# paulvantieghem/curla

Measured on AMD Instinct MI355X. Metric: SAC+CURL gradient updates/sec, batch=512 84x84x9, higher is better.
Workload: dtype f32

## Files before the change

curla_amd/_lib.py:

```python
import ctypes
import os

_HERE = os.path.dirname(os.path.abspath(__file__))
LIB_PATH = os.environ.get("CURLA_LIB_PATH") or os.path.join(_HERE, "libcurla_hip.so")

c_int, c_ll, c_float, c_size_t, vp = ctypes.c_int, ctypes.c_longlong, ctypes.c_float, ctypes.c_size_t, ctypes.c_void_p
c_u64 = ctypes.c_ulonglong
c_double = ctypes.c_double

ABI_VERSION = 8

SIGNATURES = {
    "curla_conv1_fwd": [vp, c_int, vp, vp, vp, vp, vp, vp, c_int, c_int, c_int, c_int, c_int, c_int, c_int, c_float, vp],
    "curla_conv3x3_s1_fwd": [vp, vp, vp, vp, c_int, c_int, c_int, c_int, vp],
    "curla_conv3x3_s1_fwd2": [vp, vp, vp, vp, c_int, vp, vp, vp, vp, c_int, c_int, c_int, c_int, vp],
    "curla_conv3x3_s1_fwd_stack": [c_int, vp, vp, vp, vp, c_int, vp, vp, vp, vp, c_int, c_int, c_int, c_int, vp],
    "curla_conv3x3_s1_stack_granule": [],
    "curla_conv1_fwd2": [vp, vp, vp, vp, vp, vp, vp, c_int, vp, vp, vp, vp, vp, vp, c_int, c_int, c_int, c_int, c_int, c_int,
                         c_int, c_float, vp],
    "curla_conv3x3_s1_dgrad": [vp, vp, vp, vp, c_int, c_int, c_int, c_int, vp],
    "curla_conv3x3_s1_wgrad": [vp, vp, vp, vp, vp, c_int, c_int, c_int, c_int, vp],
    "curla_conv1_wgrad": [vp, c_int, vp, vp, vp, vp, vp, vp, vp, c_int, c_int, c_int, c_int, c_int, c_int, c_int,
                          c_float, vp],
    "curla_conv3x3_s1_wgrad_slabs": [vp, vp, vp, c_int, c_int, c_int, c_int, vp, vp],
# ... 13 lines not shown
    "curla_fc_bwd_ln2": [vp, vp, vp, vp, vp, c_int, c_int, c_int, vp, c_int, vp, vp, vp, vp, c_int, c_int, vp, vp],
    "curla_curl_head": [vp, vp, vp, vp, vp, vp, c_int, c_int, vp, vp, vp, vp, vp, vp, vp, vp, vp, vp],
    "curla_gemm_nested": [vp, c_int, c_int, c_ll, c_ll, vp, c_int, c_int, c_ll, c_ll, vp, c_int, c_ll, c_ll, c_int, c_int, c_int,
                          c_int, c_int, c_float, vp, c_ll, c_ll, c_int, vp, c_int, c_ll, c_ll, vp],
    "curla_mlp_out_fwd_nested": [vp, c_ll, c_ll, vp, c_ll, c_ll, vp, c_ll, c_ll, vp, c_ll, c_ll, c_int, c_int, c_int, c_int, c_int,
                                 vp],
    "curla_gemm_multi": [c_int, vp, vp, vp, c_int, c_int, c_int, c_int, c_int, c_int, c_int, c_ll, vp],
    "curla_fc_fwd_multi": [c_int, vp, vp, vp, c_int, c_int, c_int, c_int, c_ll, c_int, vp],
    "curla_splitk_reduce": [vp, c_int, c_ll, c_int, c_int, c_int, vp, c_int, vp, c_int, vp],
    "curla_mlp_out_fwd": [vp, c_ll, vp, c_ll, vp, c_ll, vp, c_ll, c_int, c_int, c_int, c_int, vp],
    "curla_mlp_out_bwd": [vp, c_ll, vp, c_ll, vp, c_ll, vp, c_ll, vp, c_ll, c_int, c_int, c_int, c_int, vp],
    "curla_mlp_out_bwd_loss": [vp, vp, c_ll, vp, c_ll, vp, c_ll, vp, c_ll, c_int, c_int, vp, vp, c_ll, vp],
    "curla_mlp_out_bwd_bias": [vp, c_ll, vp, c_ll, vp, c_ll, vp, c_ll, vp, c_ll, c_int, c_int, c_int, c_int, vp, vp, c_ll,
                               vp],
    "curla_gemm_small_shape": [c_int, c_int, c_int, c_int],
    "curla_gemm_colsum": [vp, c_int, c_int, c_ll, vp, c_int, c_int, c_ll, vp, c_int, c_ll, c_int, c_int, c_int, c_int, vp,
                          c_ll, vp],
    "curla_linear_bwd": [vp, c_ll, vp, c_ll, vp, c_ll, vp, c_ll, vp, c_ll, vp, c_ll, vp, c_ll, c_int, c_int, c_int, c_int, vp],
    "curla_fc_ln_fwd": [vp, c_int, c_ll, c_int, vp, vp, vp, c_int, c_int, c_float, vp, vp, vp, vp, c_int, vp, vp, c_int,
                        vp],
    "curla_critic_td_loss": [vp, vp, c_ll, vp, vp, vp, vp, c_float, c_int, vp, vp, vp, vp],
    "curla_soft_update2": [vp, vp, c_size_t, c_size_t, c_float, c_float, c_float, c_float, vp],
    "curla_adam_step": [vp, vp, vp, vp, c_size_t, c_double, c_double, c_double, c_double, c_ll, vp, vp],
    "curla_adam_step_lerp": [vp, vp, vp, vp, c_size_t, c_double, c_double, c_double, c_double, c_ll, vp, vp, c_size_t,
                             c_float, c_float, c_float, c_float, vp],
    "curla_adam_step_scalar64": [vp, vp, vp, vp, c_size_t, c_double, c_double, c_double, c_double, c_ll, vp, vp, vp, vp, vp,
                                 c_double, c_double, c_double, c_double, c_ll, vp, vp],
    "curla_adam_step2": [vp, vp, vp, vp, vp, vp, c_size_t, c_size_t, c_double, c_double, c_double, c_double, c_ll, c_double,
                         c_double, c_double, c_double, c_ll, vp, vp],
    "curla_f64_pack": [vp, vp, vp],
# ... 27 lines not shown
    "curla_stage_frames_u8": [vp, vp, c_ll, c_int, c_int, c_int, c_int, c_int, c_int, c_int, c_int, vp],
    "curla_gather_stacks": [vp, vp, c_int, vp, c_int, c_int, c_int, c_int, vp, vp],
    "curla_nhwc_to_nchw": [vp, vp, c_int, c_int, c_int, c_int, vp],
    "curla_color_jiggle": [vp, vp, vp, vp, c_int, c_int, c_int, c_int, vp, vp],
    "curla_noisy_cover": [vp, vp, vp, c_float, c_float, c_float, c_int, c_int, c_int, c_int, c_int, c_int, vp, vp],
    "curla_gather_nhwc": [vp, vp, c_int, c_int, c_int, c_int, vp, vp],
    "curla_noisy_cover_rng": [vp, vp, c_float, c_u64, c_u64, vp, c_float, c_float, c_float, vp, c_int, c_int, c_int, c_int,
                              c_int, c_int, vp, vp, vp],
    "curla_color_jiggle_nchw": [vp, vp, vp, c_int, c_int, c_int, c_int, vp, vp],
    "curla_noisy_cover_nchw": [vp, vp, c_float, c_float, c_float, c_int, c_int, c_int, c_int, c_int, c_int, vp, vp],
    "curla_version": [],
    "curla_abi_version": [],
    "curla_set_option": [ctypes.c_char_p, ctypes.c_char_p],
    "curla_get_option": [ctypes.c_char_p],
}
_RESTYPES = {"curla_conv_wgrad_workspace_floats": c_size_t, "curla_version": ctypes.c_char_p,
             "curla_get_option": ctypes.c_char_p}
_ERRORS = {-1: "CURLA_ERR_ARG (bad pointer/size/alignment)", -2: "CURLA_ERR_LAUNCH (HIP launch failed)",
           -3: "CURLA_ERR_UNSUPPORTED (shape not supported by the gfx950 kernels)"}


class CurlaHipError(RuntimeError):
    pass


_lib = None


def load():
    global _lib
    if _lib is not None:
# ... 90 lines not shown
```

curla_amd/csrc/gemm.hip:

```cpp
#include <stdlib.h>
#include <string.h>

#include "common.h"
#include "options.h"

namespace {

constexpr int BM = 64, BN = 64, BK = 32;
constexpr int RSTR = BK + 8;
#ifndef CURLA_GEMM_KSTR
#define CURLA_GEMM_KSTR (BM + 4)
#endif
constexpr int KSTR = CURLA_GEMM_KSTR;
constexpr int kB3RowBytes = 64;
__device__ __forceinline__ int b3_swz(int row) { return (-((row >> 2) & 3)) & 3; }
constexpr int b3_part_bytes(int rows) { return rows * kB3RowBytes; }
constexpr int b3_tile_floats(int rows) { return 3 * b3_part_bytes(rows) / 4; }
constexpr int kGemmTileFloatsF32 = (BK * KSTR > BM * RSTR) ? BK * KSTR : BM * RSTR;
constexpr int gemm_tile_floats(int rows) {
  return rows > 64 ? b3_tile_floats(rows) : (b3_tile_floats(64) > kGemmTileFloatsF32 ? b3_tile_floats(64) : kGemmTileFloatsF32);
}

struct GemmArgs {
  const float* A;
// ... 3 lines not shown
  const float* mask;
  int M, N, K, lda, ldb, ldc, ldmask;
  long long sA, sB, sC, sBias, sMask, sSplit;
  int nbatch, ksplit, kchunk;
  float alpha;
  int relu, vecA, vecB;
  int stream_c;
  int nb_inner;
  long long sA2, sB2, sC2, sBias2, sMask2;
  float* colsum;
  long long sColsum, sColsum2;
  int nptr;
  const float* Ap[4];
  const float* Bp[4];
  float* Cp[4];
};

template <bool KMAJOR, int ROWS>
__device__ __forceinline__ void tile_load(const float* __restrict__ P, int ld, int rows_total, int r0, int k0, int kend,
                                          int vec, int tid, f32x4 (&reg)[ROWS / 32]) {
#pragma unroll
  for (int u = 0; u < ROWS / 32; ++u) {
    f32x4 v = {0, 0, 0, 0};
    if (!KMAJOR) {
      const int row = (tid >> 3) + 32 * u, k4 = (tid & 7) * 4;
      const int gr = r0 + row, gk = k0 + k4;
      if (gr < rows_total) {
        const float* p = P + (size_t)gr * ld + gk;
        if (vec && gk + 3 < kend) {
          v = *reinterpret_cast<const f32x4*>(p);
        } else {
// ... 141 lines not shown
    const float r0 = x0 - __builtin_bit_cast(float, hh << 16), r1 = x1 - __builtin_bit_cast(float, hh & 0xFFFF0000u);
    const unsigned mm = g_cvt_pk_bf16(r0, r1);
    const float s0 = r0 - __builtin_bit_cast(float, mm << 16), s1 = r1 - __builtin_bit_cast(float, mm & 0xFFFF0000u);
    o.h[p] = hh, o.m[p] = mm, o.l[p] = g_cvt_pk_bf16(s0, s1);
  }
  return o;
}

__device__ __forceinline__ f32x4 g_mfma_bf16(const gu32x4 a, const gu32x4 b, const f32x4 c) {
  return __builtin_amdgcn_mfma_f32_16x16x32_bf16(__builtin_bit_cast(gbf16x8, a), __builtin_bit_cast(gbf16x8, b), c, 0, 0, 0);
}

template <int ROWS>
using GemmLds = float[2][gemm_tile_floats(ROWS)];

template <bool AK, bool BKM, int TBM, int TBN, bool FAST, bool B3 = false, int NT = 256>
__device__ __forceinline__ void gemm_tile(const GemmArgs& g, const int bx, const int by, const int z, float (*As)[gemm_tile_floats(TBM)],
                                          float (*Bs)[gemm_tile_floats(TBN)]) {
  static_assert(!B3 || FAST, "the bf16x3 form takes interior, aligned tiles only");
  static_assert(TBM <= 64 || B3, "tiles of more than 64 rows exist in the bf16x3 form only");
  static_assert(NT == 256 || B3, "the f32 forms are written for 256 threads");
  constexpr int WR = NT / 128;
  constexpr int WM = TBM / WR;
  constexpr int MI = WM / 16;
  constexpr int RA = TBM * 8 / NT, RB = TBN * 8 / NT;
  constexpr int NJ = TBN / 32;
  constexpr int WN = TBN / 2;
  const int tid = threadIdx.x, lane = tid & 63, wave = tid >> 6;
  const int li = lane & 15, kq = lane >> 4;
  const int wm = wave >> 1, wn = wave & 1;
  const int batch = z / g.ksplit, ks = z - batch * g.ksplit;
  const int m0 = by * TBM, n0 = bx * TBN;
  const int bo = batch / g.nb_inner, bi = batch - bo * g.nb_inner;
  const float* A = g.nptr ? g.Ap[batch] : g.A + bi * g.sA + bo * g.sA2;
  const float* B = g.nptr ? g.Bp[batch] : g.B + bi * g.sB + bo * g.sB2;
  float* C = (g.nptr ? g.Cp[batch] : g.C + bi * g.sC + bo * g.sC2) + ks * g.sSplit;
  const int kbeg = ks * g.kchunk;
  const int kend = min(g.K, kbeg + g.kchunk);

  const bool epi = g.ksplit == 1;
  const float* bias = (epi && g.bias) ? g.bias + bi * g.sBias + bo * g.sBias2 : nullptr;
  const float* mask = (epi && g.mask) ? g.mask + bi * g.sMask + bo * g.sMask2 : nullptr;
  const bool vec_c = (g.ldc % 4 == 0) && ((reinterpret_cast<uintptr_t>(C) & 15) == 0) &&
                     (!mask || ((g.ldmask % 4 == 0) && ((reinterpret_cast<uintptr_t>(mask) & 15) == 0)));
  f32x4 mk[MI][NJ];
#pragma unroll
  for (int i = 0; i < MI; ++i)
#pragma unroll
    for (int j = 0; j < NJ; ++j) {
      mk[i][j] = f32x4{1.f, 1.f, 1.f, 1.f};
      const int m = m0 + wm * WM + i * 16 + li;
      const int n = n0 + wn * WN + j * 16 + 4 * kq;
      if (mask && vec_c && m < g.M && n + 3 < g.N) mk[i][j] = *reinterpret_cast<const f32x4*>(mask + (size_t)m * g.ldmask + n);
    }

  f32x4 acc[MI][NJ];
#pragma unroll
  for (int i = 0; i < MI; ++i)
#pragma unroll
    for (int j = 0; j < NJ; ++j) acc[i][j] = f32x4{0, 0, 0, 0};

  auto load = [&](int k0, f32x4 (&ra)[RA], f32x4 (&rb)[RB]) {
    if constexpr (B3) {
      tile_load_b3<AK, TBM, NT>(A, g.lda, g.M, m0, k0, tid, ra);
      tile_load_b3<BKM, TBN, NT>(B, g.ldb, g.N, n0, k0, tid, rb);
    } else if constexpr (FAST) {
      tile_load_fast<AK, TBM>(A, g.lda, g.M, m0, k0, tid, ra);
      tile_load_fast<BKM, TBN>(B, g.ldb, g.N, n0, k0, tid, rb);
// ... 63 lines not shown
    const int rem = ntiles - t;
    if (rem >= 3) load(k0 + 2 * BK, ra0, rb0);
    multiply(0);
    if (rem >= 2) {
      stage(1, ra1, rb1);
      __syncthreads();
      multiply(1);
    }
    if (rem >= 3) {
      stage(0, ra0, rb0);
      __syncthreads();
      multiply(0);
    }
  }

#pragma unroll
  for (int i = 0; i < MI; ++i)
#pragma unroll
    for (int j = 0; j < NJ; ++j) {
      const int m = m0 + wm * WM + i * 16 + li;
      const int n = n0 + wn * WN + j * 16 + 4 * kq;
      if (m >= g.M || n >= g.N) continue;
      f32x4 v = acc[i][j] * g.alpha;
      if (vec_c && n + 3 < g.N) {
        if (bias) {
#pragma unroll
          for (int r = 0; r < 4; ++r) v[r] += bias[n + r];
        }
        if (epi && g.relu) {
#pragma unroll
// ... 25 lines not shown
#endif
__device__ __forceinline__ int xcd_order(int b, int total) {
  return (CURLA_GEMM_XCD && (total & 7) == 0) ? (b & 7) * (total >> 3) + (b >> 3) : b;
}

template <bool AK, bool BKM, int TBM, int TBN, bool FAST, bool B3 = false, int NT = 256>
__global__ __launch_bounds__(NT) void gemm_kernel(GemmArgs g) {
  __shared__ __attribute__((aligned(16))) GemmLds<TBM> As;
  __shared__ __attribute__((aligned(16))) GemmLds<TBN> Bs;
  const int gx = (g.N + TBN - 1) / TBN, gy = (g.M + TBM - 1) / TBM;
  const int v = xcd_order(blockIdx.x, gx * gy * g.nbatch * g.ksplit);
  const int r = v / gy;
  gemm_tile<AK, BKM, TBM, TBN, FAST, B3, NT>(g, r % gx, v - r * gy, r / gx, As, Bs);
}

template <int TM1, int TN1, int TM2, int TN2, bool B3 = false, bool SECOND_FIRST = false, int NT = 256>
__global__ __launch_bounds__(NT) void gemm_pair_kernel(GemmArgs g1, GemmArgs g2, int n1, int gx1, int gy1, int gx2,
                                                        int gy2, int n2) {
  constexpr int RA = TM1 > TM2 ? TM1 : TM2, RB = TN1 > TN2 ? TN1 : TN2;
  __shared__ __attribute__((aligned(16))) GemmLds<RA> As;
  __shared__ __attribute__((aligned(16))) GemmLds<RB> Bs;
  int bid = blockIdx.x;
  if (CURLA_GEMM_XCD && ((n1 | n2) & 7) == 0) {
    const int x = bid & 7, i = bid >> 3, s1 = n1 >> 3, s2 = n2 >> 3;
    const int fst = SECOND_FIRST ? s2 : s1;
    const bool in_first = i < fst;
    const bool second = SECOND_FIRST ? in_first : !in_first;
    const int j = in_first ? i : i - fst;
    bid = second ? n1 + x * s2 + j : x * s1 + j;
  } else if (SECOND_FIRST) {
    bid = bid < n2 ? bid + n1 : bid - n2;
  }
  if (bid < n1) {
    const int r = bid / gy1;
    gemm_tile<true, true, TM1, TN1, true, B3, NT>(g1, r % gx1, bid - r * gy1, r / gx1,
                                                  reinterpret_cast<float(*)[gemm_tile_floats(TM1)]>(&As[0][0]),
                                                  reinterpret_cast<float(*)[gemm_tile_floats(TN1)]>(&Bs[0][0]));
  } else {
    bid -= n1;
    const int r = bid / gy2;
    gemm_tile<false, true, TM2, TN2, true, B3, NT>(g2, r % gx2, bid - r * gy2, r / gx2,
                                                   reinterpret_cast<float(*)[gemm_tile_floats(TM2)]>(&As[0][0]),
                                                   reinterpret_cast<float(*)[gemm_tile_floats(TN2)]>(&Bs[0][0]));
  }
}

__device__ float g_zero16[16];

constexpr int kFcMaxSteps = 16;

struct FcBwdArgs {
  const float* dz;
  const float* W;
  const float* mask;
  float* out;
  int B, F, K;
};

// ... 682 lines not shown

struct GemmPlan {
  bool small, wide, fast, b3;
  int tbm, tbn;
};

static int gemm_mfma_opt() { return curla_opt(kOptGemmMfma); }
static bool gemm_b3() { return gemm_mfma_opt() == kGemmMfmaB3; }

static bool big_tile_ok(const GemmArgs& g) {
  return gemm_mfma_opt() != kGemmMfmaF32 && g.ksplit == 1 && g.vecA && g.vecB && g.K % BK == 0 && g.K >= 4 * BK && g.M % 128 == 0 &&
         g.N % 64 == 0 && !g.colsum;
}
static long long big_tile_count(const GemmArgs& g) { return (long long)(g.M / 128) * (g.N / 64) * g.nbatch; }

static int gemm_plan(GemmArgs& g, int a_kmajor, int b_kmajor, GemmPlan& p, bool force_big = false) {
  const int M = g.M, N = g.N, K = g.K, nbatch = g.nbatch, ksplit = g.ksplit;
  p.small = ksplit == 1 && !g.bias && !g.mask && !g.relu && g.nptr == 0 && small_shape(M, N, K, nbatch);
  p.wide = false, p.fast = false, p.b3 = false, p.tbm = p.tbn = 16;
  if (g.colsum && !p.small) return CURLA_ERR_UNSUPPORTED;
  if (p.small) {
    const long long t16 = (long long)((M + 15) / 16) * ((N + 15) / 16) * nbatch;
    p.wide = t16 < 64 && K % 256 == 0;
    return CURLA_OK;
  }
  int kc = (K + ksplit - 1) / ksplit;
  kc = (kc + BK - 1) / BK * BK;
  g.kchunk = kc;
  g.stream_c = (long long)M * N * nbatch * (long long)sizeof(float) >= (32LL << 20);
  const long long cu2 = 2LL * curla_cu_count();
  const long long zb = (long long)nbatch * ksplit;
  const long long wgs64 = (long long)((N + 63) / 64) * ((M + 63) / 64) * zb;
  const long long wgs6432 = (long long)((N + 31) / 32) * ((M + 63) / 64) * zb;
  int tbm = 64, tbn = 64;
  if (wgs64 < cu2 && N > 32) tbn = 32;
  if (tbn == 32 && M <= 64 && a_kmajor && b_kmajor && 2 * wgs64 >= cu2) tbn = 64;
  if (tbn == 32 && wgs6432 < cu2 && M > 32) tbm = 32;
  const int tile_opt = curla_opt(kOptGemmTile);
  bool big = big_tile_ok(g) && (force_big || big_tile_count(g) >= curla_cu_count());
  switch (tile_opt) {
    case kGemmTile6464: tbm = 64, tbn = 64, big = false; break;
    case kGemmTile6432: tbm = 64, tbn = 32, big = false; break;
    case kGemmTile3232: tbm = 32, tbn = 32, big = false; break;
    case kGemmTile12864: big = big_tile_ok(g); break;
    default: break;
  }
  if (big) {
    p.tbm = 128, p.tbn = 64, p.fast = true, p.b3 = true;
    g.kchunk = g.K;
    return CURLA_OK;
  }
  p.tbm = tbm, p.tbn = tbn;
  p.fast = g.vecA && g.vecB && (K % BK == 0) && (g.kchunk % BK == 0) && (!a_kmajor || M % tbm == 0) &&
           (!b_kmajor || N % tbn == 0);
  p.b3 = p.fast && gemm_b3();
  return CURLA_OK;
}

static int gemm_launch(GemmArgs& g, int a_kmajor, int b_kmajor, hipStream_t st) {
  const int M = g.M, N = g.N, nbatch = g.nbatch, ksplit = g.ksplit;
  GemmPlan p;
// ... 25 lines not shown
  const bool b3 = p.b3;
#define CURLA_GEMM_LAUNCH3(AKM, BKMAJ, TM, TN, FS, B3F)                                                     \
  hipLaunchKernelGGL((gemm_kernel<AKM, BKMAJ, TM, TN, FS, B3F>), dim3(((N + TN - 1) / TN) * ((M + TM - 1) / TM) * nbatch * ksplit), \
                     dim3(256), 0, st, g)
#define CURLA_GEMM_LAUNCH2(AKM, BKMAJ, TM, TN)               \
  do {                                                       \
    if (b3)                                                  \
      CURLA_GEMM_LAUNCH3(AKM, BKMAJ, TM, TN, true, true);    \
    else if (fast)                                           \
      CURLA_GEMM_LAUNCH3(AKM, BKMAJ, TM, TN, true, false);   \
    else                                                     \
      CURLA_GEMM_LAUNCH3(AKM, BKMAJ, TM, TN, false, false);  \
  } while (0)
#define CURLA_GEMM_LAUNCH(AKM, BKMAJ)                        \
  do {                                                       \
    if (tbm == 128)                                          \
      hipLaunchKernelGGL((gemm_kernel<AKM, BKMAJ, 128, 64, true, true, 512>), dim3((N / 64) * (M / 128) * nbatch), dim3(512), 0, st, g); \
    else if (tbm == 32)                                      \
      CURLA_GEMM_LAUNCH2(AKM, BKMAJ, 32, 32);                \
    else if (tbn == 32)                                      \
      CURLA_GEMM_LAUNCH2(AKM, BKMAJ, 64, 32);                \
    else                                                     \
      CURLA_GEMM_LAUNCH2(AKM, BKMAJ, 64, 64);                \
  } while (0)
  if (a_kmajor && b_kmajor)
    CURLA_GEMM_LAUNCH(true, true);
  else if (a_kmajor)
    CURLA_GEMM_LAUNCH(true, false);
  else if (b_kmajor)
    CURLA_GEMM_LAUNCH(false, true);
  else
// ... 14 lines not shown
  g.A = A, g.B = B, g.C = C, g.bias = bias, g.mask = mask;
  g.M = M, g.N = N, g.K = K, g.lda = lda, g.ldb = ldb, g.ldc = ldc, g.ldmask = ldmask;
  g.sA = strideA, g.sB = strideB, g.sC = strideC, g.sBias = strideBias, g.sMask = strideMask, g.sSplit = split_stride;
  g.nbatch = nbatch, g.ksplit = ksplit;
  g.alpha = alpha, g.relu = relu;
  g.vecA = (lda % 4 == 0) && (strideA % 4 == 0) && aligned16(A);
  g.vecB = (ldb % 4 == 0) && (strideB % 4 == 0) && aligned16(B);
  g.nptr = 0;
  g.colsum = nullptr, g.sColsum = g.sColsum2 = 0;
  g.nb_inner = nbatch, g.sA2 = g.sB2 = g.sC2 = g.sBias2 = g.sMask2 = 0;
  return gemm_launch(g, a_kmajor, b_kmajor, static_cast<hipStream_t>(stream));
}

int curla_gemm_small_shape(int M, int N, int K, int nbatch) { return small_shape(M, N, K, nbatch) ? 1 : 0; }

int curla_gemm_colsum(const float* A, int a_kmajor, int lda, long long strideA, const float* B, int b_kmajor, int ldb,
                      long long strideB, float* C, int ldc, long long strideC, int M, int N, int K, int nbatch,
                      float* colsum, long long strideColsum, void* stream) {
  CURLA_REQUIRE(A && B && C && colsum && M > 0 && N > 0 && K > 0 && nbatch > 0);
  GemmArgs g;
  g.A = A, g.B = B, g.C = C, g.bias = nullptr, g.mask = nullptr;
  g.M = M, g.N = N, g.K = K, g.lda = lda, g.ldb = ldb, g.ldc = ldc, g.ldmask = 0;
  g.sA = strideA, g.sB = strideB, g.sC = strideC, g.sBias = 0, g.sMask = 0, g.sSplit = 0;
  g.nbatch = nbatch, g.ksplit = 1;
  g.alpha = 1.f, g.relu = 0;
  g.vecA = (lda % 4 == 0) && (strideA % 4 == 0) && aligned16(A);
  g.vecB = (ldb % 4 == 0) && (strideB % 4 == 0) && aligned16(B);
  g.nptr = 0;
  g.nb_inner = nbatch, g.sA2 = g.sB2 = g.sC2 = g.sBias2 = g.sMask2 = 0;
  g.colsum = colsum, g.sColsum = strideColsum, g.sColsum2 = 0;
// ... 16 lines not shown

int curla_linear_bwd(const float* dy, long long stride_dy, const float* x, long long stride_x, const float* W,
                     long long stride_W, const float* mask, long long stride_mask, float* dW, long long stride_dW,
                     float* db, long long stride_db, float* dx, long long stride_dx, int B, int N, int K, int nbatch,
                     void* stream) {
  CURLA_REQUIRE(dy && x && W && dW && dx && B > 0 && N > 0 && K > 0 && nbatch > 0);
  hipStream_t st = static_cast<hipStream_t>(stream);
  GemmArgs g1, g2;
  gemm_args_plain(g1, dy, N, stride_dy, x, K, stride_x, dW, K, stride_dW, N, K, B, nbatch);
  g1.colsum = db, g1.sColsum = stride_db;
  gemm_args_plain(g2, dy, N, stride_dy, W, K, stride_W, dx, K, stride_dx, B, K, N, nbatch);
  g2.mask = mask, g2.ldmask = K, g2.sMask = stride_mask;
  GemmPlan p1, p2;
  const bool split = curla_opt(kOptLinearBwd) == kLinearBwdSplit;
  const bool both_big = !split && big_tile_ok(g1) && big_tile_ok(g2) && big_tile_count(g1) + big_tile_count(g2) >= curla_cu_count();
  int rc = gemm_plan(g1, 1, 1, p1, both_big);
  if (rc != CURLA_OK) return rc;
  rc = gemm_plan(g2, 0, 1, p2, both_big);
  if (rc != CURLA_OK) return rc;
  const int T1 = p1.small ? 16 : 0, T2 = p2.small ? 16 : 0;
  const int gx1 = (g1.N + (T1 ? T1 : p1.tbn) - 1) / (T1 ? T1 : p1.tbn), gy1 = (g1.M + (T1 ? T1 : p1.tbm) - 1) / (T1 ? T1 : p1.tbm);
  const int gx2 = (g2.N + (T2 ? T2 : p2.tbn) - 1) / (T2 ? T2 : p2.tbn), gy2 = (g2.M + (T2 ? T2 : p2.tbm) - 1) / (T2 ? T2 : p2.tbm);
  const long long n1 = (long long)gx1 * gy1 * nbatch, n2 = (long long)gx2 * gy2 * nbatch;
  if (!split && n1 + n2 < (1LL << 30)) {
    if (p1.small && p2.small && !p1.wide && !p2.wide) {
      hipLaunchKernelGGL((gemm_small_pair_kernel<4, 8>), dim3((unsigned)(n1 + n2)), dim3(256), 0, st, g1, g2, (int)n1, gx1,
                         gy1, gx2, gy2);
      return curla_launch_status();
    }
    if (!p1.small && !p2.small && p1.fast && p2.fast && p1.tbm == 128 && p2.tbm == 128) {
      if (g2.K >= g1.K)
        hipLaunchKernelGGL((gemm_pair_kernel<128, 64, 128, 64, true, true, 512>), dim3((unsigned)(n1 + n2)), dim3(512), 0, st, g1,
                           g2, (int)n1, gx1, gy1, gx2, gy2, (int)n2);
// ... 246 lines not shown
```

curla_amd/csrc/options.h:

```cpp
#pragma once

enum CurlaOpt {
  kOptConv1U8 = 0,
  kOptConv1F32,
  kOptS1Fwd,
  kOptBwdSplit,
  kOptGemmTile,
  kOptLinearBwd,
  kOptGemmMfma,
  kOptS1Wgrad,
  kOptWgrad1U8,
  kOptCount
};

enum Conv1U8Opt { kConv1U8Auto, kConv1U8Hybrid, kConv1U8Band, kConv1U8Rw, kConv1U8Rwb, kConv1U8Values };
enum Conv1F32Opt { kConv1F32Rw, kConv1F32Band, kConv1F32Values };
enum S1FwdOpt { kS1FwdAuto, kS1FwdF23, kS1FwdF43, kS1FwdB3, kS1FwdValues };
enum BwdSplitOpt { kBwdSplitAuto, kBwdSplitOff, kBwdSplitOn, kBwdSplitValues };
enum GemmTileOpt { kGemmTileAuto, kGemmTile6464, kGemmTile6432, kGemmTile3232, kGemmTile12864, kGemmTileValues };
enum LinearBwdOpt { kLinearBwdPair, kLinearBwdSplit, kLinearBwdValues };
enum GemmMfmaOpt { kGemmMfmaAuto, kGemmMfmaF32, kGemmMfmaB3, kGemmMfmaValues };
enum S1WgradOpt { kS1WgradAuto, kS1WgradX, kS1WgradXY, kS1WgradValues };
enum Wgrad1U8Opt { kWgrad1U8Auto, kWgrad1U8F32, kWgrad1U8B16, kWgrad1U8Values };

int curla_opt(int id);
```

curla_amd/csrc/options.hip:

```cpp
#include "options.h"

#include <atomic>
#include <cctype>
#include <cstdlib>
#include <cstring>
#include <mutex>

#include "../../include/curla_hip.h"

namespace {

struct OptDef {
  const char* name;
  const char* values[6];
  const char* alias[6];
};

constexpr OptDef kDefs[kOptCount] = {
    {"conv1_u8", {"auto", "hybrid", "band", "rw", "rwb", nullptr}, {nullptr, nullptr, nullptr, nullptr, nullptr, nullptr}},
    {"conv1_f32", {"rw", "band", nullptr}, {nullptr, nullptr, nullptr}},
    {"s1_fwd", {"auto", "f23", "f43", "b3", nullptr}, {nullptr, nullptr, nullptr, "bf16x3", nullptr}},
    {"bwd_split", {"auto", "0", "1", nullptr}, {nullptr, "off", "on", nullptr}},
    {"gemm_tile", {"auto", "6464", "6432", "3232", "12864", nullptr}, {nullptr, "64x64", "64x32", "32x32", "128x64", nullptr}},
    {"linear_bwd", {"pair", "split", nullptr}, {nullptr, nullptr, nullptr}},
    {"gemm_mfma", {"auto", "f32", "b3", nullptr}, {nullptr, nullptr, "bf16x3", nullptr}},
    {"s1_wgrad", {"auto", "x", "xy", nullptr}, {nullptr, "1d", "2d", nullptr}},
    {"wgrad1_u8", {"auto", "f32", "b16", nullptr}, {nullptr, nullptr, "bf16", nullptr}},
};

constexpr int kValueCount[kOptCount] = {kConv1U8Values, kConv1F32Values, kS1FwdValues, kBwdSplitValues, kGemmTileValues,
                                        kLinearBwdValues, kGemmMfmaValues, kS1WgradValues, kWgrad1U8Values};
constexpr bool value_counts_match() {
  for (int id = 0; id < kOptCount; ++id)
    if (!kDefs[id].values[kValueCount[id] - 1] || kDefs[id].values[kValueCount[id]]) return false;
  return true;
}
static_assert(value_counts_match(), "options.h names a different number of values than kDefs lists for some option");

std::atomic<int> g_value[kOptCount];
std::once_flag g_once;

int parse(const OptDef& d, const char* text) {
  for (int i = 0; i < 6 && d.values[i]; ++i)
    if (!strcmp(text, d.values[i]) || (d.alias[i] && !strcmp(text, d.alias[i]))) return i;
  return -1;
}
// ... 47 lines not shown
```

curla_amd/curl_sac.py:

```python
import os
import warnings

import numpy as np
import torch
import torch.nn as nn

from . import autograd, ops
from .augmentations import RandomCrop
from .encoder import CNNEncoder
from .ops import ObsRef
from .optim import FlatAdam

LOG_FREQ = 25_000


def weight_init(m):
    if isinstance(m, nn.Linear):
        nn.init.orthogonal_(m.weight.data)
        if m.bias is not None:
            m.bias.data.zero_()
        return
    if isinstance(m, (nn.Conv2d, nn.ConvTranspose2d)):
        kh, kw = m.weight.shape[2:]
        assert kh == kw, "square kernels only"
# ... 213 lines not shown
class _Workspace:

    def __init__(self, agent, B):
        enc = agent.critic.encoder
        dev = agent.device
        F, A, H, L = enc.feature_dim, agent.action_dim, agent.hidden_dim, enc.num_layers
        f = lambda *shape: torch.empty(shape, device=dev, dtype=torch.float32)
        shapes = [(B, h, w, enc.num_filters) for (h, w) in enc.layer_hw[1:]]
        self.acts_pair = [f(2 * s[0], *s[1:]) for s in shapes]
        self.acts_main = [a[:B] for a in self.acts_pair]
        self.acts_tmp = [f(*s) for s in shapes]
        gmax = max(int(np.prod(s)) for s in shapes)
        self.gbuf = [f(gmax), f(gmax)]
        self.gviews = [[g[:int(np.prod(s))].view(s) for s in shapes] for g in self.gbuf]
        self.wg_ws = [f(ops.wgrad_workspace_floats(enc.obs_shape[0] if i == 0 else enc.num_filters)) for i in range(L)]
        self.z_a, self.z_t, self.z_c, self.z_pos = f(B, F), f(B, F), f(B, F), f(B, F)
        self.xhat_c, self.rstd_c, self.xhat_a, self.rstd_a = f(B, F), f(B), f(B, F), f(B)
        self.dz, self.dfc = f(B, F), f(B, F)
        self.ln_partial = f(ops.ln_partial_floats(B, F))
        self.w_partial = f(max(1, B // 16) * F * F) if ops.curl_head_supported(B, F) else None
        self.fc_out = f(B, F)
        self.a_h1, self.a_h2, self.a_out = f(B, H), f(B, H), f(B, 2 * A)
        self.a_dh1, self.a_dh2, self.a_dout = f(B, H), f(B, H), f(B, 2 * A)
        self.noise = f(B, A)
        self.mu, self.pi, self.log_std, self.tanh_ls, self.gpi = f(B, A), f(B, A), f(B, A), f(B, A), f(B, A)
        self.log_pi = f(B, 1)
        self.xa2, self.q_h1_2, self.q_h2_2, self.q2 = f(2, B, F + A), f(2, 2, B, H), f(2, 2, B, H), f(2, 2, B, 1)
        self.xa, self.q_h1, self.q_h2 = self.xa2[1], self.q_h1_2[1], self.q_h2_2[1]
        self.tq, self.q = self.q2[0], self.q2[1]
        self.dxa = f(2, B, F + A)
# ... 1053 lines not shown
```

curla_amd/ops.py:

```python
import ctypes

import torch

from . import _lib
from ._lib import call, ptr, stream

F32 = torch.float32


def _dev(t, dtype=F32):
    if not ((t.is_cuda or _lib._trace_hook is not None) and t.dtype == dtype and t.is_contiguous()):
        raise _lib.CurlaHipError(f"expected a contiguous {dtype} CUDA tensor, got {t.dtype} {t.device} "
                                 f"contiguous={t.is_contiguous()}")
    return t


class ObsRef:

    __slots__ = ("src", "is_u8", "idx", "h1", "w1", "B", "C", "Hs", "Ws", "Hc", "Wc", "guard", "pair")

    def __init__(self):
        self.guard = None
        self.pair = None

# ... 179 lines not shown
def gemm(A, a_kmajor, lda, sA, Bm, b_kmajor, ldb, sB, C, ldc, sC, M, N, K, nbatch=1, ksplit=1, split_stride=0,
         alpha=1.0, bias=None, sBias=0, relu=0, mask=None, ldmask=0, sMask=0):
    call("curla_gemm", ptr(A), a_kmajor, lda, sA, ptr(Bm), b_kmajor, ldb, sB, ptr(C), ldc, sC, M, N, K, nbatch, ksplit,
         split_stride, alpha, ptr(bias), sBias, relu, ptr(mask), ldmask, sMask, stream())


def gemm_multi(As, Bs, Cs, M, N, K, ksplit=1, split_stride=0):
    import ctypes
    n = len(As)
    P = ctypes.c_void_p * n
    a, b, c = P(*[ptr(t) for t in As]), P(*[ptr(t) for t in Bs]), P(*[ptr(t) for t in Cs])
    call("curla_gemm_multi", n, ctypes.addressof(a), ctypes.addressof(b), ctypes.addressof(c), K, K, N, M, N, K, ksplit,
         split_stride, stream())


FC_FWD_MAX_SPLIT = 64


def fc_fwd_supported(B, F_, K):
    return 50 <= F_ <= 64 and F_ % 2 == 0 and B % 128 == 0 and K % 32 == 0 and B * K * 4 < 2 ** 31 and F_ * K * 4 < 2 ** 31


def fc_fwd_nsplit(nprob, B, K):
    cap = 2 * cu_count()
    per = nprob * (B // 128)
    ns = max(1, min(FC_FWD_MAX_SPLIT, (3 * cap // 2) // per, K // 32))
    while ns > 1 and ns * per > cap and 0 < (ns * per) % cap <= cap // 8:
        ns -= 1
    return ns

# ... 400 lines not shown
```

include/curla_hip.h:

```cpp
#ifndef CURLA_HIP_H
#define CURLA_HIP_H

#include <stddef.h>
#include <stdint.h>

#ifdef __cplusplus
extern "C" {
#endif

#define CURLA_OK 0
#define CURLA_ERR_ARG (-1)
#define CURLA_ERR_LAUNCH (-2)
#define CURLA_ERR_UNSUPPORTED (-3)

const char* curla_version(void);

#define CURLA_ABI_VERSION 8
int curla_abi_version(void);

int curla_set_option(const char* name, const char* value);
const char* curla_get_option(const char* name);


int curla_conv1_fwd(const void* src, int src_kind, const int64_t* idx, const int32_t* h1, const int32_t* w1,
// ... 28 lines not shown
                            const float* g, float* workspace, int B, int C, int Hs, int Ws, int Hc, int Wc, int channels,
                            float scale, int* nslabs, void* stream);
int curla_conv3x3_s1_bwd_slabs(const float* in, const float* g, const float* w, float* gin, float* workspace, int B, int Hi,
                               int Wi, int channels, int* nslabs, void* stream);
int curla_conv1_dgrad(const float* g, const float* w, float* dobs, int B, int C, int H, int W, int channels,
                      float scale, void* stream);
int curla_wgrad_reduce_multi(int njobs, const float* const* slabs, const int* nslabs, const int* nw, const int* nb,
                             float* const* dw, float* const* db, void* stream);
size_t curla_conv_wgrad_workspace_floats(int cin);

int curla_gemm(const float* A, int a_kmajor, int lda, long long strideA, const float* B, int b_kmajor, int ldb,
               long long strideB, float* C, int ldc, long long strideC, int M, int N, int K, int nbatch, int ksplit,
               long long split_stride, float alpha, const float* bias, long long strideBias, int relu,
               const float* mask, int ldmask, long long strideMask, void* stream);
int curla_gemm_small_shape(int M, int N, int K, int nbatch);
int curla_gemm_colsum(const float* A, int a_kmajor, int lda, long long strideA, const float* B, int b_kmajor, int ldb,
                      long long strideB, float* C, int ldc, long long strideC, int M, int N, int K, int nbatch,
                      float* colsum, long long strideColsum, void* stream);
int curla_linear_bwd(const float* dy, long long stride_dy, const float* x, long long stride_x, const float* W,
                     long long stride_W, const float* mask, long long stride_mask, float* dW, long long stride_dW,
                     float* db, long long stride_db, float* dx, long long stride_dx, int B, int N, int K, int nbatch,
                     void* stream);
int curla_gemm_nested(const float* A, int a_kmajor, int lda, long long strideA, long long strideA2, const float* B,
                      int b_kmajor, int ldb, long long strideB, long long strideB2, float* C, int ldc, long long strideC,
                      long long strideC2, int M, int N, int K, int nbatch, int nbatch2, float alpha, const float* bias,
                      long long strideBias, long long strideBias2, int relu, const float* mask, int ldmask,
                      long long strideMask, long long strideMask2, void* stream);
int curla_gemm_multi(int nprob, const float* const* A, const float* const* B, float* const* C, int lda, int ldb, int ldc,
                     int M, int N, int K, int ksplit, long long split_stride, void* stream);
int curla_fc_fwd_multi(int nprob, const float* const* x, const float* const* W, float* const* partial, int B, int F, int K,
// ... 165 lines not shown
```

Measured before the change: 520.8.

## Add split-K with in-kernel last-block reduction for under-filled 128x64 GEMM pairs

Adds a split-K variant of the 128x64 bf16x3 GEMM tile. Each K-slice writes its partial accumulators to a workspace slab and bumps a per-tile atomic counter. The last arriving block sums the slabs, applies the epilogue and resets the counter. By default it is used in the linear-backward pair kernel when the two GEMMs together have fewer tiles than CUs, so the GPU is better filled. The cost is extra global traffic for the slabs, atomics and fences, and a workspace buffer reserved at agent setup.

```diff
diff --git a/curla_amd/_lib.py b/curla_amd/_lib.py
--- a/curla_amd/_lib.py
+++ b/curla_amd/_lib.py
@@ -51,6 +51,8 @@
     "curla_mlp_out_bwd_bias": [vp, c_ll, vp, c_ll, vp, c_ll, vp, c_ll, vp, c_ll, c_int, c_int, c_int, c_int, vp, vp, c_ll,
                                vp],
     "curla_gemm_small_shape": [c_int, c_int, c_int, c_int],
+    "curla_gemm_splitk_workspace": [vp, c_ll],
+    "curla_gemm_splitk_workspace_bytes": [],
     "curla_gemm_colsum": [vp, c_int, c_int, c_ll, vp, c_int, c_int, c_ll, vp, c_int, c_ll, c_int, c_int, c_int, c_int, vp,
                           c_ll, vp],
     "curla_linear_bwd": [vp, c_ll, vp, c_ll, vp, c_ll, vp, c_ll, vp, c_ll, vp, c_ll, vp, c_ll, c_int, c_int, c_int, c_int, vp],
@@ -108,7 +110,7 @@
     "curla_set_option": [ctypes.c_char_p, ctypes.c_char_p],
     "curla_get_option": [ctypes.c_char_p],
 }
-_RESTYPES = {"curla_conv_wgrad_workspace_floats": c_size_t, "curla_version": ctypes.c_char_p,
+_RESTYPES = {"curla_conv_wgrad_workspace_floats": c_size_t, "curla_gemm_splitk_workspace_bytes": c_ll, "curla_version": ctypes.c_char_p,
              "curla_get_option": ctypes.c_char_p}
 _ERRORS = {-1: "CURLA_ERR_ARG (bad pointer/size/alignment)", -2: "CURLA_ERR_LAUNCH (HIP launch failed)",
            -3: "CURLA_ERR_UNSUPPORTED (shape not supported by the gfx950 kernels)"}
diff --git a/curla_amd/csrc/gemm.hip b/curla_amd/csrc/gemm.hip
--- a/curla_amd/csrc/gemm.hip
+++ b/curla_amd/csrc/gemm.hip
@@ -41,7 +41,11 @@
   const float* Ap[4];
   const float* Bp[4];
   float* Cp[4];
+  float* sk_ws;
+  unsigned* sk_cnt;
+  int sk_s, sk_chunk, sk_slab0, sk_cnt0;
 };
+constexpr int kSkSlabFloats = 128 * 64;
 
 template <bool KMAJOR, int ROWS>
 __device__ __forceinline__ void tile_load(const float* __restrict__ P, int ld, int rows_total, int r0, int k0, int kend,
@@ -213,10 +217,11 @@
 template <int ROWS>
 using GemmLds = float[2][gemm_tile_floats(ROWS)];
 
-template <bool AK, bool BKM, int TBM, int TBN, bool FAST, bool B3 = false, int NT = 256>
+template <bool AK, bool BKM, int TBM, int TBN, bool FAST, bool B3 = false, int NT = 256, bool SK = false>
 __device__ __forceinline__ void gemm_tile(const GemmArgs& g, const int bx, const int by, const int z, float (*As)[gemm_tile_floats(TBM)],
-                                          float (*Bs)[gemm_tile_floats(TBN)]) {
+                                          float (*Bs)[gemm_tile_floats(TBN)], const int sks = 0) {
   static_assert(!B3 || FAST, "the bf16x3 form takes interior, aligned tiles only");
+  static_assert(!SK || (B3 && TBM == 128 && TBN == 64 && NT == 512), "split-K exists for the 128 x 64 bf16x3 tile");
   static_assert(TBM <= 64 || B3, "tiles of more than 64 rows exist in the bf16x3 form only");
   static_assert(NT == 256 || B3, "the f32 forms are written for 256 threads");
   constexpr int WR = NT / 128;
@@ -234,8 +239,9 @@
   const float* A = g.nptr ? g.Ap[batch] : g.A + bi * g.sA + bo * g.sA2;
   const float* B = g.nptr ? g.Bp[batch] : g.B + bi * g.sB + bo * g.sB2;
   float* C = (g.nptr ? g.Cp[batch] : g.C + bi * g.sC + bo * g.sC2) + ks * g.sSplit;
-  const int kbeg = ks * g.kchunk;
-  const int kend = min(g.K, kbeg + g.kchunk);
+  const bool split = SK && g.sk_s > 1;
+  const int kbeg = split ? sks * g.sk_chunk : ks * g.kchunk;
+  const int kend = min(g.K, kbeg + (split ? g.sk_chunk : g.kchunk));
 
   const bool epi = g.ksplit == 1;
   const float* bias = (epi && g.bias) ? g.bias + bi * g.sBias + bo * g.sBias2 : nullptr;
@@ -250,7 +256,7 @@
       mk[i][j] = f32x4{1.f, 1.f, 1.f, 1.f};
       const int m = m0 + wm * WM + i * 16 + li;
       const int n = n0 + wn * WN + j * 16 + 4 * kq;
-      if (mask && vec_c && m < g.M && n + 3 < g.N) mk[i][j] = *reinterpret_cast<const f32x4*>(mask + (size_t)m * g.ldmask + n);
+      if (!split && mask && vec_c && m < g.M && n + 3 < g.N) mk[i][j] = *reinterpret_cast<const f32x4*>(mask + (size_t)m * g.ldmask + n);
     }
 
   f32x4 acc[MI][NJ];
@@ -344,6 +350,60 @@
     }
   }
 
+  if constexpr (SK) {
+    if (split) {
+      const int gx = g.N / TBN, gy = g.M / TBM;
+      const int tile = (z * gy + by) * gx + bx;
+      f32x4* slabs = reinterpret_cast<f32x4*>(g.sk_ws) + (size_t)(g.sk_slab0 + tile * g.sk_s) * (kSkSlabFloats / 4);
+      f32x4* mine = slabs + (size_t)sks * (kSkSlabFloats / 4);
+#pragma unroll
+      for (int i = 0; i < MI; ++i)
+#pragma unroll
+        for (int j = 0; j < NJ; ++j) mine[(i * NJ + j) * NT + tid] = acc[i][j];
+      asm volatile("s_waitcnt vmcnt(0)" ::: "memory");
+      __syncthreads();
+      unsigned* cnt = g.sk_cnt + g.sk_cnt0 + tile;
+      unsigned* flag = reinterpret_cast<unsigned*>(&As[0][0]);
+      if (tid == 0) {
+        __builtin_amdgcn_fence(__ATOMIC_RELEASE, "agent");
+        asm volatile("s_waitcnt vmcnt(0)" ::: "memory");
+        *flag = __hip_atomic_fetch_add(cnt, 1u, __ATOMIC_RELAXED, __HIP_MEMORY_SCOPE_AGENT);
+      }
+      __syncthreads();
+      if (*flag != (unsigned)(g.sk_s - 1)) return;
+      if (tid == 0) {
+        __builtin_amdgcn_fence(__ATOMIC_ACQUIRE, "agent");
+        asm volatile("s_waitcnt vmcnt(0)" ::: "memory");
+        __hip_atomic_store(cnt, 0u, __ATOMIC_RELAXED, __HIP_MEMORY_SCOPE_AGENT);
+      }
+      __syncthreads();
+#pragma unroll
+      for (int i = 0; i < MI; ++i)
+#pragma unroll
+        for (int j = 0; j < NJ; ++j) {
+          const int m = m0 + wm * WM + i * 16 + li;
+          const int n = n0 + wn * WN + j * 16 + 4 * kq;
+          if (mask && vec_c) mk[i][j] = *reinterpret_cast<const f32x4*>(mask + (size_t)m * g.ldmask + n);
+        }
+      f32x4 sum[MI][NJ];
+#pragma unroll
+      for (int i = 0; i < MI; ++i)
+#pragma unroll
+        for (int j = 0; j < NJ; ++j) sum[i][j] = sks == 0 ? acc[i][j] : slabs[(i * NJ + j) * NT + tid];
+      for (int s = 1; s < g.sk_s; ++s) {
+        const f32x4* p = slabs + (size_t)s * (kSkSlabFloats / 4);
+#pragma unroll
+        for (int i = 0; i < MI; ++i)
+#pragma unroll
+          for (int j = 0; j < NJ; ++j) sum[i][j] += s == sks ? acc[i][j] : p[(i * NJ + j) * NT + tid];
+      }
+#pragma unroll
+      for (int i = 0; i < MI; ++i)
+#pragma unroll
+        for (int j = 0; j < NJ; ++j) acc[i][j] = sum[i][j];
+    }
+  }
+
 #pragma unroll
   for (int i = 0; i < MI; ++i)
 #pragma unroll
@@ -399,7 +459,17 @@
   gemm_tile<AK, BKM, TBM, TBN, FAST, B3, NT>(g, r % gx, v - r * gy, r / gx, As, Bs);
 }
 
-template <int TM1, int TN1, int TM2, int TN2, bool B3 = false, bool SECOND_FIRST = false, int NT = 256>
+template <bool AK, bool BKM>
+__global__ __launch_bounds__(512) void gemm_splitk_kernel(GemmArgs g) {
+  __shared__ __attribute__((aligned(16))) GemmLds<128> As;
+  __shared__ __attribute__((aligned(16))) GemmLds<64> Bs;
+  const int gx = g.N / 64, gy = g.M / 128;
+  const int v = xcd_order(blockIdx.x, gx * gy * g.nbatch * g.sk_s);
+  const int t = v / g.sk_s, r = t / gy;
+  gemm_tile<AK, BKM, 128, 64, true, true, 512, true>(g, r % gx, t - r * gy, r / gx, As, Bs, v - t * g.sk_s);
+}
+
+template <int TM1, int TN1, int TM2, int TN2, bool B3 = false, bool SECOND_FIRST = false, int NT = 256, bool SK = false>
 __global__ __launch_bounds__(NT) void gemm_pair_kernel(GemmArgs g1, GemmArgs g2, int n1, int gx1, int gy1, int gx2,
                                                         int gy2, int n2) {
   constexpr int RA = TM1 > TM2 ? TM1 : TM2, RB = TN1 > TN2 ? TN1 : TN2;
@@ -417,16 +487,20 @@
     bid = bid < n2 ? bid + n1 : bid - n2;
   }
   if (bid < n1) {
+    int sks = 0;
+    if (SK && g1.sk_s > 1) sks = bid % g1.sk_s, bid /= g1.sk_s;
     const int r = bid / gy1;
-    gemm_tile<true, true, TM1, TN1, true, B3, NT>(g1, r % gx1, bid - r * gy1, r / gx1,
-                                                  reinterpret_cast<float(*)[gemm_tile_floats(TM1)]>(&As[0][0]),
-                                                  reinterpret_cast<float(*)[gemm_tile_floats(TN1)]>(&Bs[0][0]));
+    gemm_tile<true, true, TM1, TN1, true, B3, NT, SK>(g1, r % gx1, bid - r * gy1, r / gx1,
+                                                      reinterpret_cast<float(*)[gemm_tile_floats(TM1)]>(&As[0][0]),
+                                                      reinterpret_cast<float(*)[gemm_tile_floats(TN1)]>(&Bs[0][0]), sks);
   } else {
     bid -= n1;
+    int sks = 0;
+    if (SK && g2.sk_s > 1) sks = bid % g2.sk_s, bid /= g2.sk_s;
     const int r = bid / gy2;
-    gemm_tile<false, true, TM2, TN2, true, B3, NT>(g2, r % gx2, bid - r * gy2, r / gx2,
-                                                   reinterpret_cast<float(*)[gemm_tile_floats(TM2)]>(&As[0][0]),
-                                                   reinterpret_cast<float(*)[gemm_tile_floats(TN2)]>(&Bs[0][0]));
+    gemm_tile<false, true, TM2, TN2, true, B3, NT, SK>(g2, r % gx2, bid - r * gy2, r / gx2,
+                                                       reinterpret_cast<float(*)[gemm_tile_floats(TM2)]>(&As[0][0]),
+                                                       reinterpret_cast<float(*)[gemm_tile_floats(TN2)]>(&Bs[0][0]), sks);
   }
 }
 
@@ -1139,8 +1213,54 @@
 }
 static long long big_tile_count(const GemmArgs& g) { return (long long)(g.M / 128) * (g.N / 64) * g.nbatch; }
 
-static int gemm_plan(GemmArgs& g, int a_kmajor, int b_kmajor, GemmPlan& p, bool force_big = false) {
+constexpr int kSkMaxDevices = 16;
+constexpr long long kSkCounterBytes = 4096;
+constexpr int kSkMinK = 128;
+struct SkWorkspace {
+  char* base;
+  long long bytes;
+};
+static SkWorkspace g_sk_ws[kSkMaxDevices];
+
+static SkWorkspace sk_workspace() {
+  int dev = 0;
+  if (hipGetDevice(&dev) != hipSuccess || dev < 0 || dev >= kSkMaxDevices) return SkWorkspace{nullptr, 0};
+  return g_sk_ws[dev];
+}
+static long long sk_bytes(long long slabs) { return kSkCounterBytes + slabs * kSkSlabFloats * (long long)sizeof(float); }
+
+static int sk_splits(int K, long long tiles, long long want, int* chunk) {
+  *chunk = K;
+  if (tiles <= 0 || tiles >= want) return 1;
+  int S = (int)((want + tiles - 1) / tiles);
+  if (S > K / kSkMinK) S = K / kSkMinK;
+  if (S < 2) return 1;
+  int kc = ((K + S - 1) / S + BK - 1) / BK * BK;
+  S = (K + kc - 1) / kc;
+  if (S < 2) return 1;
+  *chunk = kc;
+  return S;
+}
+
+static void sk_none(GemmArgs& g) { g.sk_ws = nullptr, g.sk_cnt = nullptr, g.sk_s = 1, g.sk_chunk = g.K, g.sk_slab0 = g.sk_cnt0 = 0; }
+
+static int select_splitk(GemmArgs& g) {
+  sk_none(g);
+  if (curla_opt(kOptGemmSplitK) != kGemmSplitKAll || curla_opt(kOptGemmTile) != kGemmTileAuto || !big_tile_ok(g)) return 1;
+  const long long tiles = big_tile_count(g), cu = curla_cu_count();
+  int chunk;
+  const int S = sk_splits(g.K, tiles, cu, &chunk);
+  if (S < 2 || tiles * S < cu || tiles > kSkCounterBytes / 4) return 1;
+  const SkWorkspace w = sk_workspace();
+  if (!w.base || w.bytes < sk_bytes(tiles * S)) return 1;
+  g.sk_cnt = reinterpret_cast<unsigned*>(w.base), g.sk_ws = reinterpret_cast<float*>(w.base + kSkCounterBytes);
+  g.sk_s = S, g.sk_chunk = chunk;
+  return S;
+}
+
+static int gemm_plan(GemmArgs& g, int a_kmajor, int b_kmajor, GemmPlan& p, bool force_big = false, bool allow_sk = true) {
   const int M = g.M, N = g.N, K = g.K, nbatch = g.nbatch, ksplit = g.ksplit;
+  sk_none(g);
   p.small = ksplit == 1 && !g.bias && !g.mask && !g.relu && g.nptr == 0 && small_shape(M, N, K, nbatch);
   p.wide = false, p.fast = false, p.b3 = false, p.tbm = p.tbn = 16;
   if (g.colsum && !p.small) return CURLA_ERR_UNSUPPORTED;
@@ -1170,6 +1290,7 @@
     case kGemmTile12864: big = big_tile_ok(g); break;
     default: break;
   }
+  if (!big && allow_sk && select_splitk(g) > 1) big = true;
   if (big) {
     p.tbm = 128, p.tbn = 64, p.fast = true, p.b3 = true;
     g.kchunk = g.K;
@@ -1225,7 +1346,9 @@
   } while (0)
 #define CURLA_GEMM_LAUNCH(AKM, BKMAJ)                        \
   do {                                                       \
-    if (tbm == 128)                                          \
+    if (tbm == 128 && g.sk_s > 1)                            \
+      hipLaunchKernelGGL((gemm_splitk_kernel<AKM, BKMAJ>), dim3((N / 64) * (M / 128) * nbatch * g.sk_s), dim3(512), 0, st, g); \
+    else if (tbm == 128)                                     \
       hipLaunchKernelGGL((gemm_kernel<AKM, BKMAJ, 128, 64, true, true, 512>), dim3((N / 64) * (M / 128) * nbatch), dim3(512), 0, st, g); \
     else if (tbm == 32)                                      \
       CURLA_GEMM_LAUNCH2(AKM, BKMAJ, 32, 32);                \
@@ -1270,6 +1393,18 @@
 
 int curla_gemm_small_shape(int M, int N, int K, int nbatch) { return small_shape(M, N, K, nbatch) ? 1 : 0; }
 
+int curla_gemm_splitk_workspace(void* buf, long long bytes) {
+  CURLA_REQUIRE((buf && bytes >= kSkCounterBytes && aligned16(buf)) || (!buf && bytes == 0));
+  int dev = 0;
+  CURLA_REQUIRE(hipGetDevice(&dev) == hipSuccess && dev >= 0 && dev < kSkMaxDevices);
+  g_sk_ws[dev] = SkWorkspace{static_cast<char*>(buf), bytes};
+  return CURLA_OK;
+}
+
+long long curla_gemm_splitk_workspace_bytes(void) {
+  return sk_bytes(2LL * curla_cu_count());
+}
+
 int curla_gemm_colsum(const float* A, int a_kmajor, int lda, long long strideA, const float* B, int b_kmajor, int ldb,
                       long long strideB, float* C, int ldc, long long strideC, int M, int N, int K, int nbatch,
                       float* colsum, long long strideColsum, void* stream) {
@@ -1316,9 +1451,45 @@
   GemmPlan p1, p2;
   const bool split = curla_opt(kOptLinearBwd) == kLinearBwdSplit;
   const bool both_big = !split && big_tile_ok(g1) && big_tile_ok(g2) && big_tile_count(g1) + big_tile_count(g2) >= curla_cu_count();
-  int rc = gemm_plan(g1, 1, 1, p1, both_big);
+  if (!split && !both_big && big_tile_ok(g1) && big_tile_ok(g2) && curla_opt(kOptGemmSplitK) != kGemmSplitKOff &&
+      curla_opt(kOptGemmTile) == kGemmTileAuto) {
+    const long long t1 = big_tile_count(g1), t2 = big_tile_count(g2), cu = curla_cu_count();
+    int S1 = 1, S2 = 1;
+    while (t1 * S1 + t2 * S2 < cu) {
+      const bool can1 = g1.K / (S1 + 1) >= kSkMinK, can2 = g2.K / (S2 + 1) >= kSkMinK;
+      if (!can1 && !can2) break;
+      if (can2 && (!can1 || (long long)g2.K * S1 >= (long long)g1.K * S2)) ++S2; else ++S1;
+    }
+    int c1, c2;
+    S1 = S1 > 1 ? sk_splits(g1.K, t1, t1 * S1, &c1) : (c1 = g1.K, 1);
+    S2 = S2 > 1 ? sk_splits(g2.K, t2, t2 * S2, &c2) : (c2 = g2.K, 1);
+    const long long slabs1 = S1 > 1 ? t1 * S1 : 0, slabs2 = S2 > 1 ? t2 * S2 : 0;
+    const SkWorkspace w = sk_workspace();
+    if (t1 * S1 + t2 * S2 >= cu && t1 + t2 <= kSkCounterBytes / 4 && w.base && w.bytes >= sk_bytes(slabs1 + slabs2)) {
+      GemmPlan q1, q2;
+      int rc = gemm_plan(g1, 1, 1, q1, true, false);
+      if (rc != CURLA_OK) return rc;
+      rc = gemm_plan(g2, 0, 1, q2, true, false);
+      if (rc != CURLA_OK) return rc;
+      if (!q1.small && !q2.small && q1.tbm == 128 && q2.tbm == 128) {
+      g1.sk_cnt = g2.sk_cnt = reinterpret_cast<unsigned*>(w.base);
+      g1.sk_ws = g2.sk_ws = reinterpret_cast<float*>(w.base + kSkCounterBytes);
+      g1.sk_s = S1, g1.sk_chunk = c1, g1.sk_slab0 = 0, g1.sk_cnt0 = 0;
+      g2.sk_s = S2, g2.sk_chunk = c2, g2.sk_slab0 = (int)slabs1, g2.sk_cnt0 = (int)t1;
+      const long long w1 = t1 * S1, w2 = t2 * S2;
+      if ((long long)c2 >= c1)
+        hipLaunchKernelGGL((gemm_pair_kernel<128, 64, 128, 64, true, true, 512, true>), dim3((unsigned)(w1 + w2)), dim3(512), 0, st,
+                           g1, g2, (int)w1, g1.N / 64, g1.M / 128, g2.N / 64, g2.M / 128, (int)w2);
+      else
+        hipLaunchKernelGGL((gemm_pair_kernel<128, 64, 128, 64, true, false, 512, true>), dim3((unsigned)(w1 + w2)), dim3(512), 0, st,
+                           g1, g2, (int)w1, g1.N / 64, g1.M / 128, g2.N / 64, g2.M / 128, (int)w2);
+      return curla_launch_status();
+      }
+    }
+  }
+  int rc = gemm_plan(g1, 1, 1, p1, both_big, false);
   if (rc != CURLA_OK) return rc;
-  rc = gemm_plan(g2, 0, 1, p2, both_big);
+  rc = gemm_plan(g2, 0, 1, p2, both_big, false);
   if (rc != CURLA_OK) return rc;
   const int T1 = p1.small ? 16 : 0, T2 = p2.small ? 16 : 0;
   const int gx1 = (g1.N + (T1 ? T1 : p1.tbn) - 1) / (T1 ? T1 : p1.tbn), gy1 = (g1.M + (T1 ? T1 : p1.tbm) - 1) / (T1 ? T1 : p1.tbm);
diff --git a/curla_amd/csrc/options.h b/curla_amd/csrc/options.h
--- a/curla_amd/csrc/options.h
+++ b/curla_amd/csrc/options.h
@@ -10,6 +10,7 @@
   kOptGemmMfma,
   kOptS1Wgrad,
   kOptWgrad1U8,
+  kOptGemmSplitK,
   kOptCount
 };
 
@@ -21,6 +22,7 @@
 enum LinearBwdOpt { kLinearBwdPair, kLinearBwdSplit, kLinearBwdValues };
 enum GemmMfmaOpt { kGemmMfmaAuto, kGemmMfmaF32, kGemmMfmaB3, kGemmMfmaValues };
 enum S1WgradOpt { kS1WgradAuto, kS1WgradX, kS1WgradXY, kS1WgradValues };
+enum GemmSplitKOpt { kGemmSplitKAuto, kGemmSplitKOff, kGemmSplitKAll, kGemmSplitKValues };
 enum Wgrad1U8Opt { kWgrad1U8Auto, kWgrad1U8F32, kWgrad1U8B16, kWgrad1U8Values };
 
 int curla_opt(int id);
diff --git a/curla_amd/csrc/options.hip b/curla_amd/csrc/options.hip
--- a/curla_amd/csrc/options.hip
+++ b/curla_amd/csrc/options.hip
@@ -26,10 +26,11 @@
     {"gemm_mfma", {"auto", "f32", "b3", nullptr}, {nullptr, nullptr, "bf16x3", nullptr}},
     {"s1_wgrad", {"auto", "x", "xy", nullptr}, {nullptr, "1d", "2d", nullptr}},
     {"wgrad1_u8", {"auto", "f32", "b16", nullptr}, {nullptr, nullptr, "bf16", nullptr}},
+    {"gemm_splitk", {"auto", "off", "all", nullptr}, {nullptr, nullptr, nullptr, nullptr}},
 };
 
 constexpr int kValueCount[kOptCount] = {kConv1U8Values, kConv1F32Values, kS1FwdValues, kBwdSplitValues, kGemmTileValues,
-                                        kLinearBwdValues, kGemmMfmaValues, kS1WgradValues, kWgrad1U8Values};
+                                        kLinearBwdValues, kGemmMfmaValues, kS1WgradValues, kWgrad1U8Values, kGemmSplitKValues};
 constexpr bool value_counts_match() {
   for (int id = 0; id < kOptCount; ++id)
     if (!kDefs[id].values[kValueCount[id] - 1] || kDefs[id].values[kValueCount[id]]) return false;
diff --git a/curla_amd/curl_sac.py b/curla_amd/curl_sac.py
--- a/curla_amd/curl_sac.py
+++ b/curla_amd/curl_sac.py
@@ -251,6 +251,7 @@
         self.gbuf = [f(gmax), f(gmax)]
         self.gviews = [[g[:int(np.prod(s))].view(s) for s in shapes] for g in self.gbuf]
         self.wg_ws = [f(ops.wgrad_workspace_floats(enc.obs_shape[0] if i == 0 else enc.num_filters)) for i in range(L)]
+        ops.gemm_splitk_reserve()
         self.z_a, self.z_t, self.z_c, self.z_pos = f(B, F), f(B, F), f(B, F), f(B, F)
         self.xhat_c, self.rstd_c, self.xhat_a, self.rstd_a = f(B, F), f(B), f(B, F), f(B)
         self.dz, self.dfc = f(B, F), f(B, F)
diff --git a/curla_amd/ops.py b/curla_amd/ops.py
--- a/curla_amd/ops.py
+++ b/curla_amd/ops.py
@@ -217,6 +217,21 @@
          split_stride, stream())
 
 
+_SPLITK_WS = {}
+
+
+def gemm_splitk_reserve():
+    if _lib._trace_hook is not None:
+        return
+    dev = torch.cuda.current_device()
+    if dev not in _SPLITK_WS:
+        n = int(_lib.load().curla_gemm_splitk_workspace_bytes())
+        buf = torch.zeros(n, dtype=torch.uint8, device=torch.device("cuda", dev))
+        call("curla_gemm_splitk_workspace", buf.data_ptr(), n)
+        _SPLITK_WS[dev] = buf
+    return _SPLITK_WS[dev]
+
+
 FC_FWD_MAX_SPLIT = 64
 
 
diff --git a/include/curla_hip.h b/include/curla_hip.h
--- a/include/curla_hip.h
+++ b/include/curla_hip.h
@@ -66,6 +66,8 @@
                long long split_stride, float alpha, const float* bias, long long strideBias, int relu,
                const float* mask, int ldmask, long long strideMask, void* stream);
 int curla_gemm_small_shape(int M, int N, int K, int nbatch);
+int curla_gemm_splitk_workspace(void* buf, long long bytes);
+long long curla_gemm_splitk_workspace_bytes(void);
 int curla_gemm_colsum(const float* A, int a_kmajor, int lda, long long strideA, const float* B, int b_kmajor, int ldb,
                       long long strideB, float* C, int ldc, long long strideC, int M, int N, int K, int nbatch,
                       float* colsum, long long strideColsum, void* stream);
```

Measured after the change: 521.9 (median of 6 runs). No clear change (+0.2%).
